# senikm/trpx

Measured on AMD Instinct MI355X. Metric: frames/s (Terse encode + Prolix decode round trip, 512x512 uint16 stack, bit-exact vs CPU ref), higher is better.
Workload: dtype u16

## Files before the change

trpx_amd/csrc/api.hip:

```cpp
#include <hip/hip_runtime.h>
#include <stdarg.h>
#include <stdio.h>
#include <stdlib.h>
#include <string.h>
#include <algorithm>
#include <vector>

#include "../../include/trpx_hip.h"
#include "encode_kernels.hpp"
#include "profile.hpp"

namespace trpx {
Profiler& profiler() {
    static thread_local Profiler p;
    return p;
}
}

namespace {

thread_local char g_err[512] = "";
thread_local bool t_force_two_pass = false;

int fail(int code, const char* fmt, ...) {
// ... 225 lines not shown
        trpx::fused_ws_forget(workspace, workspace_bytes, ws + w.fused);
        HIP_TRY(trpx::launch_encode_fused(dtype, a, ws + w.fused, static_cast<hipStream_t>(stream)));
    } else {
        trpx::fused_ws_forget(workspace, workspace_bytes);
        HIP_TRY(trpx::launch_encode(dtype, a, static_cast<hipStream_t>(stream)));
        if (index && out)
            return build_index_impl(dtype, out, out_capacity, frame_offsets, n_values, n_frames, block, index, status, false, stream);
    }
    return TRPX_OK;
}

int trpx_encode_checked(int dtype, const void* pixels, size_t n_values, size_t n_frames, unsigned block, uint8_t* out,
                        size_t out_capacity, uint64_t* frame_offsets, uint32_t* status, void* index, void* workspace,
                        size_t workspace_bytes, void* stream, uint32_t* host_status) {
    uint32_t st[TRPX_STATUS_WORDS] = {0};
    for (int attempt = 0; attempt < 2; ++attempt) {
        t_force_two_pass = attempt == 1;
        const int rc = trpx_encode_indexed(dtype, pixels, n_values, n_frames, block, out, out_capacity, frame_offsets, status,
                                           index, workspace, workspace_bytes, stream);
        t_force_two_pass = false;
        if (rc) return rc;
        HIP_TRY(hipMemcpyAsync(st, status, sizeof st, hipMemcpyDeviceToHost, static_cast<hipStream_t>(stream)));
        HIP_TRY(hipStreamSynchronize(static_cast<hipStream_t>(stream)));
        if (st[0] != TRPX_ERR_TIMEOUT) break;
    }
    if (host_status) memcpy(host_status, st, sizeof st);
    if (st[0]) return fail((int)st[0], "trpx_encode_checked: device status %u", st[0]);
    return TRPX_OK;
}

int trpx_decode(int stream_signed, int out_dtype, const uint8_t* terse, size_t terse_bytes,
                const uint64_t* frame_offsets, size_t n_values, size_t n_frames, unsigned block, void* pixels_out,
                uint32_t* status, void* workspace, size_t workspace_bytes, void* stream) {
    trpx::FrameGeom g;
    if (!trpx_dtype_size(out_dtype)) return fail(TRPX_ERR_INVALID_ARG, "trpx_decode: unknown dtype %d", out_dtype);
    if (is64(out_dtype))
        return trpx_decode_convert(stream_signed, out_dtype, terse, terse_bytes, frame_offsets, n_values, n_frames, block, pixels_out,
                                   status, workspace, workspace_bytes, stream);
    if (block == 0 || block > kMaxBlock)
        return fail(TRPX_ERR_UNSUPPORTED, "trpx_decode: block=%u (supported: 1..%u)", block, kMaxBlock);
    if ((stream_signed != 0) != (trpx_dtype_is_signed(out_dtype) != 0))
        return fail(TRPX_ERR_UNSUPPORTED, "trpx_decode: stream signed=%d into dtype %d: only same-signedness decode "
                    "is defined by the reference (Terse.hpp:356-357)", stream_signed, out_dtype);
    if (!geom_of(n_values, block, &g) || !sizes_ok(g, n_frames) || terse_bytes == 0)
        return fail(TRPX_ERR_INVALID_ARG, "trpx_decode: bad sizes");
    if (!terse || !pixels_out || !status || !workspace) return fail(TRPX_ERR_INVALID_ARG, "trpx_decode: null pointer");
    if ((uintptr_t)terse % 4 || (uintptr_t)workspace % 8 || (uintptr_t)frame_offsets % 8 || (uintptr_t)status % 8 ||
        (uintptr_t)pixels_out % trpx_dtype_size(out_dtype))
        return fail(TRPX_ERR_INVALID_ARG, "trpx_decode: misaligned pointer (terse needs 4 B, workspace 8 B)");
    const DecWs w = dec_ws(g, n_frames, trpx_dtype_size(out_dtype));
    if (workspace_bytes < w.total)
        return fail(TRPX_ERR_CAPACITY, "trpx_decode: workspace %zu < %zu", workspace_bytes, w.total);

    trpx::fused_ws_forget(workspace, workspace_bytes);
    trpx::DecodeArgs a{};
    a.terse = terse;
    a.terse_bytes = terse_bytes;
    a.frame_offsets = frame_offsets;
    a.geom = g;
    a.n_frames = (uint32_t)n_frames;
    a.pixels_out = pixels_out;
    a.status = status;
    char* ws = static_cast<char*>(workspace);
    a.walk_offsets = reinterpret_cast<uint64_t*>(ws + w.walk_offsets);
    a.tile_off = reinterpret_cast<uint64_t*>(ws + w.tile_off);
    a.widths = reinterpret_cast<uint8_t*>(ws + w.widths);
    a.seg_ws = ws + w.seg;
#ifdef TRPX_DIAGNOSTICS
    static const bool no_defer = getenv("TRPX_NO_DEFER") != nullptr;
#else
    constexpr bool no_defer = false;
#endif
    a.defer = no_defer ? nullptr : reinterpret_cast<uint32_t*>(ws + w.defer + trpx::kDeferFront);
    const int route = g_decode_path;
    const bool basic = route == 1, force_tiles = route == 2;
    const bool bits32 = 8 * (uint64_t)trpx_worst_case_bytes(out_dtype, n_values, block) < 0xF0000000ull;
    const bool fast_ok = frame_offsets && !basic && bits32 && block == (unsigned)trpx::kBlock;
    const bool frame26 = 8 * (uint64_t)trpx_worst_case_bytes(out_dtype, n_values, block) + (1u << 17) < (1ull << 26);
    a.chain = route != 4 && route != 2 && bits32;
    a.parts_per_frame = a.chain ? trpx::chain_parts_per_frame(g, n_frames, trpx_dtype_size(out_dtype)) : trpx::parts_per_frame(g, n_frames);
    const bool parts_ok = a.parts_per_frame > 1u && n_frames * (uint64_t)a.parts_per_frame < 0x7FFFFFFFull && a.defer;
    if (parts_ok) {
        a.parts = reinterpret_cast<trpx::PartDesc*>(ws + w.parts);
        a.part_ws = ws + w.part_ws;
    } else a.parts_per_frame = 1;
    if (fast_ok && (parts_ok || (frame26 && trpx::parts_per_frame(g, n_frames) == 1u)) && !force_tiles)
        HIP_TRY(trpx::launch_decode_frames(out_dtype, a, static_cast<hipStream_t>(stream)));
    else if (fast_ok)
        HIP_TRY(trpx::launch_decode_fast(out_dtype, a, false, static_cast<hipStream_t>(stream)));
    else
        HIP_TRY(trpx::launch_decode(out_dtype, a, frame_offsets != nullptr, static_cast<hipStream_t>(stream)));
    return TRPX_OK;
}

static int build_index_impl(int dtype, const uint8_t* terse, size_t terse_bytes, const uint64_t* frame_offsets,
                            size_t n_values, size_t n_frames, unsigned block, void* index, uint32_t* status,
                            bool clear_status, void* stream) {
    trpx::FrameGeom g;
    if (block != (unsigned)trpx::kBlock) return fail(TRPX_ERR_UNSUPPORTED, "trpx_build_index: the decode index needs block=12");
    if (is64(dtype)) return fail(TRPX_ERR_UNSUPPORTED, "trpx_build_index: no decode index for 64-bit containers (generic kernels)");
    if (!trpx_dtype_size(dtype) || !geom_of(n_values, block, &g) || !sizes_ok(g, n_frames) || !terse_bytes)
        return fail(TRPX_ERR_INVALID_ARG, "trpx_build_index: bad dtype/sizes");
    if (!terse || !frame_offsets || !index || !status) return fail(TRPX_ERR_INVALID_ARG, "trpx_build_index: null pointer");
    if ((uintptr_t)terse % 4 || (uintptr_t)index % 16 || (uintptr_t)frame_offsets % 8 || (uintptr_t)status % 8)
        return fail(TRPX_ERR_INVALID_ARG, "trpx_build_index: misaligned pointer");
    if (8 * (uint64_t)trpx_worst_case_bytes(dtype, n_values, block) >= 0xF0000000ull)
        return fail(TRPX_ERR_UNSUPPORTED, "trpx_build_index: frames of >= 2^32 bits");
    const IdxLayout il = idx_layout(g, n_frames, trpx_dtype_size(dtype));
    trpx::DecodeArgs a{};
    a.terse = terse;
    a.terse_bytes = terse_bytes;
    a.frame_offsets = frame_offsets;
    a.geom = g;
    a.n_frames = (uint32_t)n_frames;
    a.status = status;
    a.tile_off = reinterpret_cast<uint64_t*>(static_cast<char*>(index) + il.group_off);
    a.widths = reinterpret_cast<uint8_t*>(static_cast<char*>(index) + il.widths);
    a.seg_ws = static_cast<char*>(index) + il.seg;
    a.defer = reinterpret_cast<uint32_t*>(static_cast<char*>(index) + il.defer + trpx::kDeferFront);
    a.index_per_frame = 8 * (uint64_t)trpx_worst_case_bytes(dtype, n_values, block) + (1u << 17) < (1ull << 26) && g_decode_path != 2;
    a.parts_per_frame = trpx::chain_parts_per_frame(g, n_frames, trpx_dtype_size(dtype));
    a.chain = a.parts_per_frame > 1u && n_frames * (uint64_t)a.parts_per_frame < 0x7FFFFFFFull && g_decode_path != 2 && g_decode_path != 4;
    if (a.chain) {
        a.parts = reinterpret_cast<trpx::PartDesc*>(static_cast<char*>(index) + il.parts);
        a.part_ws = static_cast<char*>(index) + il.part_ws;
    } else a.parts_per_frame = 1;
    HIP_TRY(trpx::launch_walk_only(a, (uint32_t)(8 * trpx_dtype_size(dtype)), clear_status, static_cast<hipStream_t>(stream)));
    return TRPX_OK;
}

int trpx_build_index(int dtype, const uint8_t* terse, size_t terse_bytes, const uint64_t* frame_offsets,
                     size_t n_values, size_t n_frames, unsigned block, void* index, uint32_t* status, void* stream) {
    return build_index_impl(dtype, terse, terse_bytes, frame_offsets, n_values, n_frames, block, index, status, true, stream);
}

int trpx_decode_indexed(int stream_signed, int out_dtype, const uint8_t* terse, size_t terse_bytes,
                        const uint64_t* frame_offsets, const void* index, size_t n_values, size_t n_frames,
                        unsigned block, void* pixels_out, uint32_t* status, void* stream) {
    trpx::FrameGeom g;
    if (!trpx_dtype_size(out_dtype)) return fail(TRPX_ERR_INVALID_ARG, "trpx_decode_indexed: unknown dtype %d", out_dtype);
    if (block != (unsigned)trpx::kBlock) return fail(TRPX_ERR_UNSUPPORTED, "trpx_decode_indexed: block=%u", block);
// ... 579 lines not shown
```

trpx_amd/csrc/codec_common.hpp:

```cpp
#pragma once
#include <hip/hip_runtime.h>
#include <stdint.h>

namespace trpx {

constexpr int kBlock = 12;
constexpr int kWave = 64;
constexpr int kThreads = 256;
constexpr int kTileBlocks = kThreads;
constexpr int kTileValues = kTileBlocks * kBlock;

struct FrameGeom {
    uint64_t n_values;
    uint32_t n_blocks;
    uint32_t n_tiles;
    uint32_t block;
};

template <typename T> struct PixelTraits;
template <> struct PixelTraits<uint8_t>  { using U = uint8_t;  static constexpr int bits = 8;  static constexpr bool is_signed = false; };
template <> struct PixelTraits<int8_t>   { using U = uint8_t;  static constexpr int bits = 8;  static constexpr bool is_signed = true;  };
template <> struct PixelTraits<uint16_t> { using U = uint16_t; static constexpr int bits = 16; static constexpr bool is_signed = false; };
template <> struct PixelTraits<int16_t>  { using U = uint16_t; static constexpr int bits = 16; static constexpr bool is_signed = true;  };
template <> struct PixelTraits<uint32_t> { using U = uint32_t; static constexpr int bits = 32; static constexpr bool is_signed = false; };
// ... 49 lines not shown
        return s < 0 ? 0u - (uint32_t)s : (uint32_t)s;
    }
    return (uint32_t)(typename PixelTraits<T>::U)v;
}

__device__ __forceinline__ uint32_t wave_inclusive_scan(uint32_t v) {
    v += (uint32_t)__builtin_amdgcn_update_dpp(0, (int)v, 0x111, 0xf, 0xf, false);
    v += (uint32_t)__builtin_amdgcn_update_dpp(0, (int)v, 0x112, 0xf, 0xf, false);
    v += (uint32_t)__builtin_amdgcn_update_dpp(0, (int)v, 0x114, 0xf, 0xf, false);
    v += (uint32_t)__builtin_amdgcn_update_dpp(0, (int)v, 0x118, 0xf, 0xf, false);
    v += (uint32_t)__builtin_amdgcn_update_dpp(0, (int)v, 0x142, 0xa, 0xf, false);
    v += (uint32_t)__builtin_amdgcn_update_dpp(0, (int)v, 0x143, 0xc, 0xf, false);
    return v;
}

__device__ __forceinline__ uint32_t wave_max(uint32_t v) {
    auto step = [](uint32_t x, uint32_t y) { return x > y ? x : y; };
    v = step(v, (uint32_t)__builtin_amdgcn_update_dpp(0, (int)v, 0x111, 0xf, 0xf, false));
    v = step(v, (uint32_t)__builtin_amdgcn_update_dpp(0, (int)v, 0x112, 0xf, 0xf, false));
    v = step(v, (uint32_t)__builtin_amdgcn_update_dpp(0, (int)v, 0x114, 0xf, 0xf, false));
    v = step(v, (uint32_t)__builtin_amdgcn_update_dpp(0, (int)v, 0x118, 0xf, 0xf, false));
    v = step(v, (uint32_t)__builtin_amdgcn_update_dpp(0, (int)v, 0x142, 0xa, 0xf, false));
    v = step(v, (uint32_t)__builtin_amdgcn_update_dpp(0, (int)v, 0x143, 0xc, 0xf, false));
    return (uint32_t)__builtin_amdgcn_readlane((int)v, 63);
}

__device__ __forceinline__ int lane_id() { return (int)(threadIdx.x & 63u); }
__device__ __forceinline__ int wave_id() { return __builtin_amdgcn_readfirstlane((int)(threadIdx.x >> 6)); }

__device__ __forceinline__ uint32_t block_exclusive_scan(uint32_t v, uint32_t* wave_tot, uint32_t* total) {
    uint32_t inc = wave_inclusive_scan(v);
    if (lane_id() == 63) wave_tot[wave_id()] = inc;
    __syncthreads();
    uint32_t t0 = wave_tot[0], t1 = wave_tot[1], t2 = wave_tot[2], t3 = wave_tot[3];
    int w = wave_id();
    uint32_t base = (w > 0 ? t0 : 0u) + (w > 1 ? t1 : 0u) + (w > 2 ? t2 : 0u);
    *total = t0 + t1 + t2 + t3;
    return base + inc - v;
}

template <int kUnused = 0>
__global__ __launch_bounds__(kThreads) void k_zero_words(uint64_t* __restrict__ p, uint64_t n, uint64_t* __restrict__ q,
                                                         uint64_t m) {
    for (uint64_t i = (uint64_t)blockIdx.x * kThreads + threadIdx.x; i < n; i += (uint64_t)gridDim.x * kThreads) p[i] = 0ull;
    if (blockIdx.x == 0 && threadIdx.x < m) q[threadIdx.x] = 0ull;
}
inline void zero_status(uint32_t* status, hipStream_t st) {
    hipLaunchKernelGGL(k_zero_words<0>, dim3(1), dim3(kThreads), 0, st, static_cast<uint64_t*>(nullptr), (uint64_t)0,
                       reinterpret_cast<uint64_t*>(status), (uint64_t)4);
}

__host__ __device__ inline uint64_t align_up(uint64_t x, uint64_t a) { return (x + a - 1) / a * a; }
constexpr uint32_t kDeferSlots = 64, kDeferSlotWords = 16;
constexpr size_t kDeferFront = 8u * kDeferSlots * kDeferSlotWords;
inline size_t defer_bytes(size_t n_frames) { return kDeferFront + align_up(4 * (n_frames + 2), 256); }

}
```

trpx_amd/csrc/decode_frame.hip:

```cpp
#include "codec_common.hpp"
#include "encode_kernels.hpp"
#include "profile.hpp"
#include "unpack_common.hpp"

namespace trpx {

#ifndef TRPX_FRAME_WAVES
#define TRPX_FRAME_WAVES 4
#endif
constexpr int kFrameWaves = TRPX_FRAME_WAVES;
constexpr int kFrameThreads = kFrameWaves * kWave;

#ifndef TRPX_FRAME_CHUNK_DW
#define TRPX_FRAME_CHUNK_DW 2048
#endif
#ifndef TRPX_IDX_TOUCH
#define TRPX_IDX_TOUCH 1
#endif
template <typename T>
struct FrameCfg {
#ifdef TRPX_FRAME_GPW
    static constexpr int kGpw = TRPX_FRAME_GPW;
#else
    static constexpr int kGpw = 4;
#endif
    static constexpr int kStepGroups = (kFrameWaves - 1) * kGpw;
    static constexpr int kStepBlocks = kStepGroups * kWave;
    static constexpr int kChunkDw = TRPX_FRAME_CHUNK_DW;
#ifdef TRPX_DEC_DIRECT_STORES
    static constexpr bool kOutStaged = sizeof(T) == 4;
#else
    static constexpr bool kOutStaged = true;
#endif
    static constexpr int kRawDw = 4 * RawQuads<T>::n;
    static constexpr int kOutDw = kWave * kBlock * (int)sizeof(T) / 4;
    static_assert(kChunkDw % (kWave * 4) == 0, "window = whole 1 KB pieces");
};

__device__ __forceinline__ void lds_dma16(const uint32_t* src_uniform, uint32_t lane_byte_offset, uint32_t lds_base) {
    uint32_t keep;
    asm volatile("s_mov_b32 %0, m0\n\ts_mov_b32 m0, %3\n\ts_nop 0\n\tglobal_load_lds_dwordx4 %1, %2\n\ts_mov_b32 m0, %0"
                 : "=&s"(keep) : "v"(lane_byte_offset), "s"(src_uniform), "s"(lds_base) : "memory");
}

template <typename T, int MODE, bool PARTS = false, bool LINES = false>
__device__ __forceinline__ void decode_frame_body(const uint8_t* __restrict__ terse, uint64_t terse_bytes,
                                                  const uint64_t* __restrict__ frame_offsets, const FrameGeom& g,
                                                  T* __restrict__ pixels_out, uint32_t* __restrict__ defer,
                                                  uint32_t* __restrict__ status, const uint64_t item,
                                                  const uint8_t* __restrict__ idx_widths, const uint64_t* __restrict__ idx_group_off,
                                                  const PartDesc* __restrict__ parts = nullptr) {
    using Cfg = FrameCfg<T>;
    constexpr bool IDX = MODE == 1;
    constexpr int kStepBlocks = Cfg::kStepBlocks, kChunkDw = Cfg::kChunkDw;
    constexpr uint32_t kMaxW = PixelTraits<T>::bits;
    __shared__ __attribute__((aligned(16))) uint32_t s_chunk[kChunkDw + 4];
    constexpr int kPosEntries = kStepBlocks + 64 + 68;
    __shared__ uint32_t s_pos[2][kPosEntries];
    uint32_t* const s_posx = &s_pos[0][0];
    constexpr uint32_t kPosBits = 26, kPosMask = (1u << kPosBits) - 1u;
    __shared__ __attribute__((aligned(16))) uint32_t s_out[kFrameWaves - 1][Cfg::kOutStaged ? Cfg::kOutDw + kStageCarryDw : 4];
    __shared__ uint32_t s_err;
#ifdef TRPX_DEC_LDS_PAD
    __shared__ uint32_t s_pad[TRPX_DEC_LDS_PAD / 4];
    if (terse_bytes == 1) s_pad[threadIdx.x] = 0;
#endif
    __shared__ uint32_t s_role[kFrameWaves];
    __shared__ uint64_t s_keep[3];

    const uint32_t lane = (uint32_t)lane_id();
    const int hw_wave = wave_id();
    uint64_t frame = item;
    uint32_t pb0 = 0, pb1 = g.n_blocks, ppos0 = 0, pw0 = 0, ppos1 = 0, pw1 = 0;
    if constexpr (PARTS && MODE == 1) {
        const uint32_t unit_blocks = (uint32_t)(uintptr_t)parts;
        const uint32_t upf = (g.n_blocks + unit_blocks - 1u) / unit_blocks;
        frame = item / upf;
        pb0 = (uint32_t)(item % upf) * unit_blocks;
        pb1 = pb0 + unit_blocks < g.n_blocks ? pb0 + unit_blocks : g.n_blocks;
        ppos0 = (uint32_t)idx_group_off[frame * g.n_tiles + pb0 / (uint32_t)kTileBlocks];
        pw0 = pb0 ? (uint32_t)idx_widths[frame * g.n_blocks + pb0 - 1u] : 0u;
        if (pb1 < g.n_blocks) {
            ppos1 = (uint32_t)idx_group_off[frame * g.n_tiles + pb1 / (uint32_t)kTileBlocks];
            pw1 = (uint32_t)idx_widths[frame * g.n_blocks + pb1 - 1u];
        }
    } else if constexpr (PARTS) {
        const PartDesc d = parts[item];
        frame = d.frame; pb0 = d.b0; pb1 = d.b1; ppos0 = d.pos0; pw0 = d.w0; ppos1 = d.pos1; pw1 = d.w1;
        if (pb1 <= pb0) return;
    }
    const uint64_t fo = frame_offsets[frame], fe = frame_offsets[frame + 1];
    if (threadIdx.x == 0) {
        s_err = (fe > fo && fe <= terse_bytes && (uint64_t)ppos0 < 8 * (fe - fo) && pb1 <= g.n_blocks) ? 0u : 1u;
        s_keep[0] = (uint64_t)(uintptr_t)status; s_keep[1] = (uint64_t)(uintptr_t)defer; s_keep[2] = item;
    }
    uint32_t hw_slot = 0;
    {
        uint32_t hwid;
        asm volatile("s_getreg_b32 %0, hwreg(HW_REG_HW_ID)" : "=s"(hwid));
        if (lane == 0) s_role[hw_wave] = ((hwid >> 4) & 3u) == (hwid & 3u) ? 1u : 0u;
        hw_slot = hwid & 7u;
    }
    __syncthreads();
    int walker_wave = 0;
#pragma unroll
    for (int i = kFrameWaves - 1; i >= 0; --i) walker_wave = s_role[i] ? i : walker_wave;
    walker_wave = __builtin_amdgcn_readfirstlane(walker_wave);
    const int wave = (hw_wave - walker_wave + kFrameWaves) % kFrameWaves;
    if (s_err) {
        if (threadIdx.x == 0) atomicMax(&status[0], 5u);
        return;
    }
    const uint32_t* __restrict__ s32 = reinterpret_cast<const uint32_t*>(terse);
    const uint64_t n_dw = (terse_bytes + 3) / 4;
    const bool base16 = ((uintptr_t)terse & 15) == 0;
    const uint64_t frame_abit = 8 * fo + ppos0;
    const uint32_t limit = (uint32_t)(8 * (fe - fo) - ppos0);
    const uint64_t frame_dw = frame_abit >> 5;
    const uint32_t frame_sh = (uint32_t)(frame_abit & 31);
    const uint32_t n_blocks = pb1 - pb0;
    const bool at_end = pb1 == g.n_blocks;
    const uint32_t nb_last = at_end ? (uint32_t)(g.n_values - (uint64_t)(g.n_blocks - 1) * kBlock) : (uint32_t)kBlock;
    const uint32_t sb0 = defer ? (uint32_t)((kFrameWaves - 1) * kWave) : (uint32_t)kStepBlocks;
    const uint32_t n_steps = n_blocks <= sb0 ? 1u : 1u + (n_blocks - sb0 + kStepBlocks - 1) / kStepBlocks;
    auto step_begin = [&](uint32_t t) -> uint32_t { return t == 0u ? 0u : sb0 + (t - 1u) * kStepBlocks; };
    T* __restrict__ fout = pixels_out + frame * g.n_values + (uint64_t)pb0 * kBlock;
    const uint32_t out_c = LINES ? (uint32_t)((uintptr_t)fout & 127u) : 0u;

#ifdef TRPX_DEC_NO_STORE
    uint32_t diag_acc = 0;
#endif
    int32_t c_lo = 0, c_hi = 0;
    uint32_t b = 0, w_prev = pw0, pos = 0;
#ifndef TRPX_DEC_WALK_PRIO
#define TRPX_DEC_WALK_PRIO 3
#endif
#ifndef TRPX_DEFER_NUM
#define TRPX_DEFER_NUM 2
#define TRPX_DEFER_DEN 9
#endif
    if (wave == 0) __builtin_amdgcn_s_setprio(TRPX_DEC_WALK_PRIO);
    constexpr int kIdxChunks = IDX ? kStepBlocks / kWave : 1;
    constexpr int kIdxQuads = IDX ? kStepBlocks / (4 * kWave) : 1;
    static_assert(!IDX || kStepBlocks % (4 * kWave) == 0, "the width prefetch covers a super-step in whole quads of 64 lanes (TRPX_FRAME_GPW: a multiple of 4 per three extraction waves)");
    __shared__ __attribute__((aligned(4))) uint8_t s_wnext[IDX ? kStepBlocks : 4];
    [[maybe_unused]] auto idx_load = [&](uint32_t ss, uint32_t (&dst)[kIdxQuads]) {
        const uint8_t* __restrict__ wfl = idx_widths + frame * g.n_blocks + pb0;
        const uint32_t bb = step_begin(ss), be = step_begin(ss + 1u) < n_blocks ? step_begin(ss + 1u) : n_blocks;
#pragma unroll
        for (int j = 0; j < kIdxQuads; ++j) {
            const uint32_t bi = bb + 4u * ((uint32_t)j * kWave + lane);
            uint32_t v = 0u;
            if (bi + 4u <= be) __builtin_memcpy(&v, wfl + bi, 4);
            else {
#pragma unroll
                for (uint32_t k = 0; k < 4u; ++k) v |= bi + k < be ? (uint32_t)wfl[bi + k] << (8u * k) : 0u;
            }
            dst[j] = v;
        }
    };
    [[maybe_unused]] auto idx_park = [&](const uint32_t (&src)[kIdxQuads]) {
#pragma unroll
        for (int j = 0; j < kIdxQuads; ++j) reinterpret_cast<uint32_t*>(s_wnext)[j * kWave + lane] = src[j];
    };
    if constexpr (IDX) {
// ... 373 lines not shown
                        uint32_t ss = sq;
                        asm volatile("" : "+v"(ss));
                        if (mine) UnpackRegsDispatch<T, 0, PixelTraits<T>::bits>::run(raw, ss, wd, o);
                        todo &= ~__ballot(mine);
                    }
#ifdef TRPX_DEC_NO_STORE
                    if (full) diag_acc ^= o[0];
#else
                    if (full) store_packed<T>(dst, o);
#endif
                }
                if (blk + 1 == n_blocks && blk < step1 && !full) {
                    const uint32_t mask = w >= 32u ? 0xFFFFFFFFu : ((1u << w) - 1u);
                    uint32_t p = q;
                    for (uint32_t k = 0; k < nb_last; ++k) {
                        uint32_t f = 0;
                        if (w) {
                            const uint64_t d = frame_dw + (p >> 5);
                            const uint64_t two = (uint64_t)(d < n_dw ? s32[d] : 0u) | ((uint64_t)(d + 1 < n_dw ? s32[d + 1] : 0u) << 32);
                            f = (uint32_t)(two >> (p & 31u)) & mask;
                            if (PixelTraits<T>::is_signed) f = (uint32_t)((int32_t)(f << (32u - w)) >> (32u - w));
                        }
                        dst[k] = (T)f;
                        p += w;
                    }
                }
            }
        }
#ifdef TRPX_DEC_STAMPS
        { const uint64_t t1 = __builtin_readcyclecounter(); st_work += t1 - st_t0; st_t0 = t1; }
#endif
        __syncthreads();
#ifdef TRPX_DEC_STAMPS
        { const uint64_t t1 = __builtin_readcyclecounter(); st_wait += t1 - st_t0; st_t0 = t1; }
#endif
        if (s_err) break;
    }
#ifdef TRPX_DEC_STAMPS
    if (lane == 0) {
        uint32_t hwid;
        asm volatile("s_getreg_b32 %0, hwreg(HW_REG_HW_ID)" : "=s"(hwid));
        uint32_t* dbg = reinterpret_cast<uint32_t*>(fout) + 8 * wave;
        dbg[0] = (uint32_t)st_work; dbg[1] = (uint32_t)st_wait; dbg[2] = hwid; dbg[3] = (uint32_t)(st_t0 - st_start);
        dbg[4] = (uint32_t)(st_start & 0xFFFFFFFFu);
        uint32_t xcc;
        asm volatile("s_getreg_b32 %0, hwreg(HW_REG_XCC_ID)" : "=s"(xcc));
        dbg[5] = xcc;
        dbg[6] = dbg[7] = 0;
    }
#endif
#ifdef TRPX_DEC_NO_STORE
    if (diag_acc == 0x12345678u) fout[threadIdx.x] = (T)diag_acc;
#endif
    if (threadIdx.x == 0 && s_err != 0u) {
        asm volatile("" ::: "memory");
        uint32_t* const status_l = reinterpret_cast<uint32_t*>((uintptr_t)s_keep[0]);
        uint32_t* const defer_l = reinterpret_cast<uint32_t*>((uintptr_t)s_keep[1]);
        if (s_err == 1u) atomicMax(&status_l[0], 5u);
        if (s_err >= 2u) {
            defer_l[1u + atomicAdd(&defer_l[0], 1u)] = (uint32_t)s_keep[2] | (s_err == 3u ? 0x80000000u : 0u);
            if (s_err == 3u) atomicAdd(reinterpret_cast<unsigned long long*>(defer_l) - 2, 1ull);
        }
    }
}

template <typename T, bool LINES>
__global__ __launch_bounds__(kFrameThreads, sizeof(T) == 4 ? 6 : 8) void k_decode_frames(const uint8_t* __restrict__ terse, uint64_t terse_bytes,
                                                               const uint64_t* __restrict__ frame_offsets, FrameGeom g,
                                                               T* __restrict__ pixels_out, uint32_t* __restrict__ defer,
                                                               uint32_t* __restrict__ status) {
    decode_frame_body<T, 0, false, LINES>(terse, terse_bytes, frame_offsets, g, pixels_out, defer, status, blockIdx.x, nullptr, nullptr);
}

template <typename T>
__global__ __launch_bounds__(kFrameThreads, sizeof(T) == 4 ? 6 : 8) void k_decode_parts(const uint8_t* __restrict__ terse, uint64_t terse_bytes,
                                                               const uint64_t* __restrict__ frame_offsets, FrameGeom g,
                                                               T* __restrict__ pixels_out, uint32_t* __restrict__ status,
                                                               const PartDesc* __restrict__ parts, const uint32_t* __restrict__ frame_mode) {
    if (status[0] != 0u) return;
    if (frame_mode && frame_mode[parts[blockIdx.x].frame] != 0u) return;
    decode_frame_body<T, 0, true, true>(terse, terse_bytes, frame_offsets, g, pixels_out, nullptr, status, blockIdx.x, nullptr, nullptr, parts);
}

template <typename T>
__global__ __launch_bounds__(kFrameThreads, sizeof(T) == 4 ? 6 : 8) void k_decode_frames_indexed(const uint8_t* __restrict__ terse, uint64_t terse_bytes,
                                                               const uint64_t* __restrict__ frame_offsets, FrameGeom g,
                                                               const uint8_t* __restrict__ widths, const uint64_t* __restrict__ group_off,
                                                               const uint32_t* __restrict__ list, T* __restrict__ pixels_out,
                                                               uint32_t* __restrict__ status) {
    uint64_t frame = blockIdx.x;
    if (list) {
        if (blockIdx.x >= list[0] || status[0] != 0u) return;
        frame = list[1u + blockIdx.x] & 0x7FFFFFFFu;
    }
#ifdef TRPX_IDX_LINES
    decode_frame_body<T, 1, false, true>(terse, terse_bytes, frame_offsets, g, pixels_out, nullptr, status, frame, widths, group_off);
#else
    decode_frame_body<T, 1>(terse, terse_bytes, frame_offsets, g, pixels_out, nullptr, status, frame, widths, group_off);
#endif
}

template <typename T>
__global__ __launch_bounds__(kFrameThreads, sizeof(T) == 4 ? 6 : 8) void k_decode_units_indexed(const uint8_t* __restrict__ terse, uint64_t terse_bytes,
                                                               const uint64_t* __restrict__ frame_offsets, FrameGeom g,
                                                               const uint8_t* __restrict__ widths, const uint64_t* __restrict__ group_off,
                                                               uint32_t unit_blocks, T* __restrict__ pixels_out, uint32_t* __restrict__ status,
                                                               const uint32_t* __restrict__ frame_mode) {
    if (status[0] != 0u) return;
    if (frame_mode && frame_mode[blockIdx.x / ((g.n_blocks + unit_blocks - 1u) / unit_blocks)] == 0u) return;
    decode_frame_body<T, 1, true>(terse, terse_bytes, frame_offsets, g, pixels_out, nullptr, status, blockIdx.x, widths, group_off,
                                  reinterpret_cast<const PartDesc*>((uintptr_t)unit_blocks));
}
template <typename T>
static uint32_t units_choose(const DecodeArgs& a, uint64_t* cost_out);
template <typename T>
static hipError_t launch_decode_units_indexed_t(const DecodeArgs& a, hipStream_t st, const uint32_t* frame_mode) {
    const uint32_t unit_blocks = units_choose<T>(a, nullptr);
    const uint32_t upf = (a.geom.n_blocks + unit_blocks - 1u) / unit_blocks;
    hipLaunchKernelGGL((k_decode_units_indexed<T>), dim3(a.n_frames * upf), dim3(kFrameThreads), 0, st, a.terse, (uint64_t)a.terse_bytes,
                       a.frame_offsets, a.geom, static_cast<const uint8_t*>(a.widths), static_cast<const uint64_t*>(a.tile_off), unit_blocks,
                       static_cast<T*>(a.pixels_out), a.status, frame_mode);
    return hipGetLastError();
}
constexpr uint64_t units_resident(size_t pixel_bytes) { return (uint64_t)(pixel_bytes == 4 ? 6 : 8) * 256u; }
// ... 31 lines not shown
                                                               uint32_t* __restrict__ defer, uint32_t* __restrict__ status) {
    decode_frame_body<T, 2>(terse, terse_bytes, frame_offsets, g, static_cast<T*>(nullptr), defer, status, blockIdx.x, widths, group_off);
}

hipError_t launch_index_frames(uint32_t max_w, const DecodeArgs& a, bool clear_status, hipStream_t st) {
    hipLaunchKernelGGL(k_zero_words<0>, dim3(1), dim3(kThreads), 0, st, reinterpret_cast<uint64_t*>(a.defer) - kDeferSlots * kDeferSlotWords,
                       (uint64_t)(kDeferSlots * kDeferSlotWords + 1), reinterpret_cast<uint64_t*>(a.status), (uint64_t)(clear_status ? 4 : 0));
    if (max_w <= 8u)
        hipLaunchKernelGGL((k_index_frames<uint8_t>), dim3(a.n_frames), dim3(kFrameThreads), 0, st, a.terse, (uint64_t)a.terse_bytes,
                           a.frame_offsets, a.geom, a.widths, a.tile_off, a.defer, a.status);
    else if (max_w <= 16u)
        hipLaunchKernelGGL((k_index_frames<uint16_t>), dim3(a.n_frames), dim3(kFrameThreads), 0, st, a.terse, (uint64_t)a.terse_bytes,
                           a.frame_offsets, a.geom, a.widths, a.tile_off, a.defer, a.status);
    else
        hipLaunchKernelGGL((k_index_frames<uint32_t>), dim3(a.n_frames), dim3(kFrameThreads), 0, st, a.terse, (uint64_t)a.terse_bytes,
                           a.frame_offsets, a.geom, a.widths, a.tile_off, a.defer, a.status);
    return launch_seg_listed(a, max_w, st);
}

template <typename T>
static hipError_t launch_decode_frames_indexed_t(const DecodeArgs& a, const uint32_t* list, hipStream_t st) {
#ifdef TRPX_IDX_AS_UNITS
    if (!list) return launch_decode_units_indexed_t<T>(a, st, nullptr);
#endif
    if (!list && a.geom.n_blocks > 8u * FrameCfg<T>::kStepBlocks) {
        uint64_t cost_units = 0;
        units_choose<T>(a, &cost_units);
        const uint64_t resident = units_resident(sizeof(T));
        const uint64_t cost_whole = ((a.n_frames + resident - 1) / resident) * ((uint64_t)a.geom.n_blocks + FrameCfg<T>::kStepBlocks);
        if (10u * cost_units < 9u * cost_whole) return launch_decode_units_indexed_t<T>(a, st, nullptr);
    }
    hipLaunchKernelGGL((k_decode_frames_indexed<T>), dim3(a.n_frames), dim3(kFrameThreads), 0, st, a.terse, (uint64_t)a.terse_bytes,
                       a.frame_offsets, a.geom, static_cast<const uint8_t*>(a.widths), static_cast<const uint64_t*>(a.tile_off), list,
                       static_cast<T*>(a.pixels_out), a.status);
    return hipGetLastError();
}

hipError_t launch_decode_frames_indexed(int dtype, const DecodeArgs& a, const uint32_t* list, hipStream_t st) {
    switch (dtype) {
    case 0: return launch_decode_frames_indexed_t<uint8_t>(a, list, st);
    case 1: return launch_decode_frames_indexed_t<int8_t>(a, list, st);
    case 2: return launch_decode_frames_indexed_t<uint16_t>(a, list, st);
    case 3: return launch_decode_frames_indexed_t<int16_t>(a, list, st);
    case 4: return launch_decode_frames_indexed_t<uint32_t>(a, list, st);
    case 5: return launch_decode_frames_indexed_t<int32_t>(a, list, st);
    }
    return hipErrorInvalidValue;
}

template <typename T>
static hipError_t launch_decode_frames_t(const DecodeArgs& a, hipStream_t st) {
    uint32_t* defer = a.defer && a.seg_ws ? a.defer : nullptr;
    const bool chain = a.chain && a.parts && a.parts_per_frame > 1u;
    if (chain) {
        if (!defer) return hipErrorInvalidValue;
        const hipError_t e = launch_chain_zero(a, (uint32_t)PixelTraits<T>::bits, true, st);
        if (e != hipSuccess) return e;
    } else
        hipLaunchKernelGGL(k_zero_words<0>, dim3(1), dim3(kThreads), 0, st,
                           defer ? reinterpret_cast<uint64_t*>(defer) - kDeferSlots * kDeferSlotWords : static_cast<uint64_t*>(nullptr),
                           (uint64_t)(defer ? kDeferSlots * kDeferSlotWords + 1 : 0),
                           reinterpret_cast<uint64_t*>(a.status), (uint64_t)4);
    Profiler& prof = profiler();
    prof.begin();
    prof.mark(st);
    if (chain) {
        if (!defer) return hipErrorInvalidValue;
        constexpr int dt = PixelTraits<T>::bits == 8 ? (PixelTraits<T>::is_signed ? 1 : 0)
                           : PixelTraits<T>::bits == 16 ? (PixelTraits<T>::is_signed ? 3 : 2) : (PixelTraits<T>::is_signed ? 5 : 4);
        constexpr bool narrow = sizeof(T) < 4;
        const uint32_t* frame_mode = nullptr;
        hipError_t e = launch_build_index_chain(a, (uint32_t)PixelTraits<T>::bits, narrow, &frame_mode, st);
        if (e != hipSuccess) return e;
        prof.mark(st);
        e = launch_seg_listed(a, (uint32_t)PixelTraits<T>::bits, st);
        if (e != hipSuccess) return e;
#ifdef TRPX_CHAIN_EXTRACT_TILES
        const bool tiles = TRPX_CHAIN_EXTRACT_TILES != 0;
#else
        const bool tiles = sizeof(T) == 4 || a.geom.n_blocks < (1u << 18);
#endif
        e = tiles ? launch_unpack_tiles(dt, a, st, narrow ? frame_mode : nullptr) : launch_decode_units_indexed(dt, a, st, narrow ? frame_mode : nullptr);
        if (e != hipSuccess) return e;
        if constexpr (narrow)
            hipLaunchKernelGGL((k_decode_parts<T>), dim3(a.n_frames * a.parts_per_frame), dim3(kFrameThreads), 0, st, a.terse, (uint64_t)a.terse_bytes,
                               a.frame_offsets, a.geom, static_cast<T*>(a.pixels_out), a.status, static_cast<const PartDesc*>(a.parts), frame_mode);
        prof.mark(st);
        return hipGetLastError();
    } else if (a.parts && a.parts_per_frame > 1u) {
        if (!defer) return hipErrorInvalidValue;
        const hipError_t e = launch_build_parts(a, (uint32_t)PixelTraits<T>::bits, st);
        if (e != hipSuccess) return e;
        hipLaunchKernelGGL((k_decode_parts<T>), dim3(a.n_frames * a.parts_per_frame), dim3(kFrameThreads), 0, st, a.terse, (uint64_t)a.terse_bytes,
                           a.frame_offsets, a.geom, static_cast<T*>(a.pixels_out), a.status, static_cast<const PartDesc*>(a.parts),
                           static_cast<const uint32_t*>(nullptr));
    } else if ((a.geom.n_values * sizeof(T)) % 128u == 0u && (uintptr_t)a.pixels_out % 128u == 0u)
        hipLaunchKernelGGL((k_decode_frames<T, false>), dim3(a.n_frames), dim3(kFrameThreads), 0, st, a.terse, (uint64_t)a.terse_bytes,
                           a.frame_offsets, a.geom, static_cast<T*>(a.pixels_out), defer, a.status);
    else
        hipLaunchKernelGGL((k_decode_frames<T, true>), dim3(a.n_frames), dim3(kFrameThreads), 0, st, a.terse, (uint64_t)a.terse_bytes,
                           a.frame_offsets, a.geom, static_cast<T*>(a.pixels_out), defer, a.status);
    prof.mark(st);
    if (defer) {
        const hipError_t e = launch_decode_deferred(PixelTraits<T>::bits == 8 ? (PixelTraits<T>::is_signed ? 1 : 0)
                                                    : PixelTraits<T>::bits == 16 ? (PixelTraits<T>::is_signed ? 3 : 2)
                                                                                 : (PixelTraits<T>::is_signed ? 5 : 4), a, st);
        prof.mark(st);
        if (e != hipSuccess) return e;
    }
    return hipGetLastError();
}

hipError_t launch_decode_frames(int dtype, const DecodeArgs& a, hipStream_t st) {
    switch (dtype) {
    case 0: return launch_decode_frames_t<uint8_t>(a, st);
    case 1: return launch_decode_frames_t<int8_t>(a, st);
    case 2: return launch_decode_frames_t<uint16_t>(a, st);
    case 3: return launch_decode_frames_t<int16_t>(a, st);
    case 4: return launch_decode_frames_t<uint32_t>(a, st);
    case 5: return launch_decode_frames_t<int32_t>(a, st);
    }
    return hipErrorInvalidValue;
}

}
```

trpx_amd/csrc/encode_fused.hip:

```cpp
#include <stddef.h>
#include <utility>
#include "codec_common.hpp"
#include "encode_kernels.hpp"
#include "profile.hpp"
#include <stdlib.h>
#include <mutex>
#include <vector>

namespace trpx {

#ifndef TRPX_FUSED_SUB32
#define TRPX_FUSED_SUB32 5
#endif
#ifndef TRPX_FUSED_SUB16
#define TRPX_FUSED_SUB16 4
#endif
template <typename T> constexpr int sub_tiles() { return sizeof(T) <= 2 ? TRPX_FUSED_SUB16 : TRPX_FUSED_SUB32; }
#ifndef TRPX_FUSED_OCC16
#define TRPX_FUSED_OCC16 8
#endif
#ifndef TRPX_FUSED_OCC32
#define TRPX_FUSED_OCC32 4
#endif
template <typename T> constexpr int fused_occupancy() { return sizeof(T) == 1 ? 8 : (sizeof(T) == 2 ? TRPX_FUSED_OCC16 : TRPX_FUSED_OCC32); }
// ... 763 lines not shown
    __syncthreads();
    if (threadIdx.x == 0) {
        uint32_t m = s_max[0];
        for (int i = 1; i < 4; ++i) m = s_max[i] > m ? s_max[i] : m;
        if (m) atomicMax(&status[1], m);
    }
    for (uint64_t i = b; i < n_frame_words; i += (uint64_t)gridDim.x * kThreads) frame_words[i] = 0ull;
    if (b == 0 && ws_tag) ws_tag[0] = tag;
    if (b >= n_tiles) return;
    tile_desc[b] = 0ull;
    if (failed || b == 0) { xw[b] = 0ull; return; }
    if (!(pw & kBndHead)) { xw[b] = 0ull; return; }
    const uint64_t d = pw & kPosMask;
    if (b > 1 && (pb & kBndHead) && (pb & kPosMask) == d) return;
    uint32_t acc = (uint32_t)xb;
    xw[b] = 0ull;
    for (uint64_t k = b + 1; k < n_tiles; ++k) {
        const uint64_t pk = pos[k];
        if (!((pk & kBndHead) && (pk & kPosMask) == d)) break;
        acc |= (uint32_t)xw[k];
        xw[k] = 0ull;
    }
    if (4 * d + 4 <= out_capacity) out32[d] = acc;
}

template <typename T>
static uint32_t fused_tiles_per_frame(const FrameGeom& g) {
    constexpr uint32_t tb = sub_tiles<T>() * kThreads;
    return (g.n_blocks + tb - 1) / tb;
}

size_t fused_workspace_bytes(const FrameGeom& g, size_t n_frames) {
    const size_t tpf = ((size_t)g.n_blocks + 2 * kThreads - 1) / (2 * kThreads);
    return align_up(8 * (3 * n_frames * tpf + 16 * ((size_t)kAccLines + 1) * n_frames + 1), 256) + 64 * n_frames * tpf;
}

namespace {
struct CleanSig {
    uint32_t elem, tiles_per_frame, n_frames, n_blocks;
    bool operator==(const CleanSig& o) const { return elem == o.elem && tiles_per_frame == o.tiles_per_frame && n_frames == o.n_frames && n_blocks == o.n_blocks; }
};
struct CleanWs { int device; const void* ptr; CleanSig sig; uint64_t tag; };
std::mutex g_clean_mu;
std::vector<CleanWs> g_clean;
uint64_t g_next_tag = 0x5452505800000001ull;
}
void fused_ws_forget(const void* lo, size_t bytes, const void* keep) {
    std::lock_guard<std::mutex> lk(g_clean_mu);
    const char* a = static_cast<const char*>(lo);
    for (size_t i = 0; i < g_clean.size();) {
        const char* p = static_cast<const char*>(g_clean[i].ptr);
        if (p != keep && (!lo || (p >= a && p < a + bytes))) { g_clean[i] = g_clean.back(); g_clean.pop_back(); } else ++i;
    }
}

template <typename T>
static hipError_t launch_fused_t(const EncodeArgs& e, void* ws, hipStream_t st) {
    FusedArgs a;
    a.g = e.geom;
    a.n_frames = e.n_frames;
    a.tiles_per_frame = fused_tiles_per_frame<T>(e.geom);
    a.out_capacity = e.out_capacity;
    const size_t tiles = (size_t)e.n_frames * a.tiles_per_frame;
    a.tile_desc = static_cast<uint64_t*>(ws);
    a.tail_desc = a.tile_desc + tiles;
    a.bnd_pos = a.tail_desc + tiles;
    a.n_acc = fused_acc_lines(a.tiles_per_frame);
    a.acc_stride = 16u * a.n_acc;
    a.frame_acc = a.bnd_pos + tiles;
    a.frame_pref = a.frame_acc + 1;
    a.frame_base = a.frame_acc + (size_t)a.acc_stride * e.n_frames;
    a.frame_offsets = e.frame_offsets;
    a.out32 = reinterpret_cast<uint32_t*>(e.out);
    a.status = e.status;
    a.idx_widths = e.idx_widths;
    a.idx_group_off = e.idx_group_off;
    const size_t frame_words = 16 * ((size_t)a.n_acc + 1) * e.n_frames;
    uint64_t* const frame_words_base = a.frame_acc;
    a.ws_tag = frame_words_base + frame_words;
    a.stamps = reinterpret_cast<uint64_t*>(static_cast<char*>(ws) + align_up(8 * (3 * tiles + frame_words + 1), 256));
#ifdef TRPX_DIAGNOSTICS
    a.debug = getenv("TRPX_FUSED_DEBUG") ? (uint32_t)atoi(getenv("TRPX_FUSED_DEBUG")) : 0u;
#else
    a.debug = 0u;
#endif
    hipStreamCaptureStatus cap = hipStreamCaptureStatusNone;
    if (hipStreamIsCapturing(st, &cap) != hipSuccess) { (void)hipGetLastError(); cap = hipStreamCaptureStatusActive; }
    const bool capturing = cap != hipStreamCaptureStatusNone;
    int device = -1;
    (void)hipGetDevice(&device);
    const CleanSig sig{(uint32_t)sizeof(T), a.tiles_per_frame, e.n_frames, e.geom.n_blocks};
    uint64_t expect = 0, tag = 0;
    if (!capturing) {
        std::lock_guard<std::mutex> lk(g_clean_mu);
        tag = g_next_tag++;
        for (size_t i = 0; i < g_clean.size(); ++i)
            if (g_clean[i].device == device && g_clean[i].ptr == ws) {
                if (g_clean[i].sig == sig) expect = g_clean[i].tag;
                g_clean[i] = g_clean.back(); g_clean.pop_back();
                break;
            }
    }
    a.expect_tag = expect;
    Profiler& prof = profiler();
    prof.begin();
    prof.mark(st);
// ... 39 lines not shown
```

trpx_amd/csrc/encode_kernels.hpp:

```cpp
#pragma once
#include <hip/hip_runtime.h>
#include <stdint.h>
#include <stddef.h>
#include "codec_common.hpp"

namespace trpx {

struct EncodeArgs {
    const void* pixels;
    FrameGeom   geom;
    uint32_t    n_frames;
    uint8_t*    out;
    size_t      out_capacity;
    uint64_t*   frame_offsets;
    uint32_t*   status;
    uint64_t*   frame_size;
    uint64_t*   tile_off;
    uint32_t*   tile_bits;
    uint8_t*    idx_widths;
    uint64_t*   idx_group_off;
};

struct PartDesc {
    uint32_t frame, b0, b1, pos0, w0, pos1, w1, pad;
};
constexpr uint32_t kPartBlocks = 16384;
constexpr uint32_t kPartMaxBlocks = 32768;
constexpr uint32_t kManyFrames = 768;
constexpr uint32_t kManyBlocks = 1u << 20;
uint32_t single_part_blocks(size_t n_frames);
void set_single_part_rule(uint32_t many_frames, uint32_t many_blocks);

struct DecodeArgs {
    const uint8_t*  terse;
    size_t          terse_bytes;
    const uint64_t* frame_offsets;
    FrameGeom       geom;
    uint32_t        n_frames;
    void*           pixels_out;
    uint32_t*       status;
    uint64_t*       tile_off;
    uint8_t*        widths;
    uint64_t*       walk_offsets;
    uint32_t*       defer;
    void*           seg_ws;
    bool            index_per_frame = false;
    PartDesc*       parts = nullptr;
    uint32_t        parts_per_frame = 1;
    void*           part_ws = nullptr;
    bool            index_given = false;
    bool            chain = false;
};
uint32_t parts_per_frame(const FrameGeom& g, size_t n_frames);
size_t part_workspace_bytes(const FrameGeom& g, size_t n_frames);
hipError_t launch_build_parts(const DecodeArgs& a, uint32_t max_w, hipStream_t st);
uint32_t chain_parts_per_frame(const FrameGeom& g, size_t n_frames, size_t pixel_bytes);
size_t chain_workspace_bytes(const FrameGeom& g, size_t n_frames, size_t pixel_bytes);
hipError_t launch_build_index_chain(const DecodeArgs& a, uint32_t max_w, bool narrow, const uint32_t** frame_mode, hipStream_t st);
hipError_t launch_chain_zero(const DecodeArgs& a, uint32_t max_w, bool clear_status, hipStream_t st);
hipError_t launch_unpack_tiles(int dtype, const DecodeArgs& a, hipStream_t st, const uint32_t* frame_mode = nullptr);

hipError_t launch_encode(int dtype, const EncodeArgs& a, hipStream_t st);
hipError_t launch_encode_generic(int dtype, const EncodeArgs& a, hipStream_t st);
size_t fused_workspace_bytes(const FrameGeom& g, size_t n_frames);
hipError_t launch_encode_fused(int dtype, const EncodeArgs& a, void* ws, hipStream_t st);
void fused_ws_forget(const void* lo, size_t bytes, const void* keep = nullptr);
hipError_t launch_decode(int dtype, const DecodeArgs& a, bool have_offsets, hipStream_t st);
hipError_t launch_decode_convert(int dtype, const DecodeArgs& a, int stream_signed, bool have_offsets, hipStream_t st);
hipError_t launch_decode_fast(int dtype, const DecodeArgs& a, bool have_index, hipStream_t st, bool per_frame = false);
hipError_t launch_decode_frames(int dtype, const DecodeArgs& a, hipStream_t st);
hipError_t launch_decode_frames_indexed(int dtype, const DecodeArgs& a, const uint32_t* list, hipStream_t st);
hipError_t launch_decode_units_indexed(int dtype, const DecodeArgs& a, hipStream_t st, const uint32_t* frame_mode = nullptr);
hipError_t launch_index_frames(uint32_t max_w, const DecodeArgs& a, bool clear_status, hipStream_t st);
hipError_t launch_seg_listed(const DecodeArgs& a, uint32_t max_w, hipStream_t st);
hipError_t launch_seg_groups(const DecodeArgs& a, uint32_t max_w, const uint64_t* states, hipStream_t st);
hipError_t launch_walk_only(const DecodeArgs& a, uint32_t max_w, bool clear_status, hipStream_t st);
hipError_t launch_walk_serial(const DecodeArgs& a, uint32_t max_w, hipStream_t st);
hipError_t launch_index_group_states(const DecodeArgs& a, uint64_t* states, hipStream_t st);
hipError_t launch_walk_groups(const DecodeArgs& a, uint32_t max_w, const uint64_t* states, bool clear_status, hipStream_t st);
size_t seg_workspace_bytes(const FrameGeom& g, size_t n_frames);
size_t dense_workspace_bytes(const FrameGeom& g, size_t n_frames);
hipError_t launch_dense_listed(const DecodeArgs& a, uint32_t max_w, void* dense_ws, const uint32_t* list, hipStream_t st);
void set_dense_route(bool on);
hipError_t launch_seg_walk(const DecodeArgs& a, uint32_t max_w, hipStream_t st);
bool seg_single_wave(const FrameGeom& g, size_t n_frames);
hipError_t launch_decode_deferred(int dtype, const DecodeArgs& a, hipStream_t st);
hipError_t launch_synth(int dtype, uint64_t seed, uint64_t frame0, size_t n_frames, size_t n_values,
                        void* out, hipStream_t st);

}
```

Baseline: 3.803 million.

## Fold decode defer-workspace zeroing into the frame kernel's last-arriving block

Removes the separate k_zero_words launch before the frame decode kernel when the workspace is known clean, tracked by a host-side tag registry. The last block to arrive, counted with a packed 64-bit atomic counter, resets the defer slots and status and writes a tag. A later call can skip zeroing if the tag matches, and falls back to a device-side reset when it does not. This saves one kernel launch per decode call. The cost is added atomic traffic, host mutex bookkeeping, and stale-tag correctness risks.

```diff
diff --git a/trpx_amd/csrc/api.hip b/trpx_amd/csrc/api.hip
--- a/trpx_amd/csrc/api.hip
+++ b/trpx_amd/csrc/api.hip
@@ -301,6 +301,13 @@
     if (workspace_bytes < w.total)
         return fail(TRPX_ERR_CAPACITY, "trpx_decode: workspace %zu < %zu", workspace_bytes, w.total);
 
+    char* ws = static_cast<char*>(workspace);
+    hipStreamCaptureStatus cap = hipStreamCaptureStatusNone;
+    if (hipStreamIsCapturing(static_cast<hipStream_t>(stream), &cap) != hipSuccess) { (void)hipGetLastError(); cap = hipStreamCaptureStatusActive; }
+    const bool capturing = cap != hipStreamCaptureStatusNone;
+    const uint32_t ws_elem = 0x100u + (uint32_t)trpx_dtype_size(out_dtype);
+    uint64_t ws_expect = 0, ws_tag = 0;
+    if (!capturing) ws_expect = trpx::clean_ws_take(ws + w.defer, ws_elem, (uint32_t)n_frames, g.n_blocks, &ws_tag);
     trpx::fused_ws_forget(workspace, workspace_bytes);
     trpx::DecodeArgs a{};
     a.terse = terse;
@@ -310,7 +317,11 @@
     a.n_frames = (uint32_t)n_frames;
     a.pixels_out = pixels_out;
     a.status = status;
-    char* ws = static_cast<char*>(workspace);
+    bool ws_clean = false;
+    a.ws_expect = ws_expect;
+    a.ws_tag = ws_tag;
+    a.ws_capturing = capturing;
+    a.ws_clean_out = &ws_clean;
     a.walk_offsets = reinterpret_cast<uint64_t*>(ws + w.walk_offsets);
     a.tile_off = reinterpret_cast<uint64_t*>(ws + w.tile_off);
     a.widths = reinterpret_cast<uint8_t*>(ws + w.widths);
@@ -333,9 +344,10 @@
         a.parts = reinterpret_cast<trpx::PartDesc*>(ws + w.parts);
         a.part_ws = ws + w.part_ws;
     } else a.parts_per_frame = 1;
-    if (fast_ok && (parts_ok || (frame26 && trpx::parts_per_frame(g, n_frames) == 1u)) && !force_tiles)
+    if (fast_ok && (parts_ok || (frame26 && trpx::parts_per_frame(g, n_frames) == 1u)) && !force_tiles) {
         HIP_TRY(trpx::launch_decode_frames(out_dtype, a, static_cast<hipStream_t>(stream)));
-    else if (fast_ok)
+        if (ws_clean && !capturing) trpx::clean_ws_put(ws + w.defer, ws_elem, (uint32_t)n_frames, g.n_blocks, ws_tag);
+    } else if (fast_ok)
         HIP_TRY(trpx::launch_decode_fast(out_dtype, a, false, static_cast<hipStream_t>(stream)));
     else
         HIP_TRY(trpx::launch_decode(out_dtype, a, frame_offsets != nullptr, static_cast<hipStream_t>(stream)));
diff --git a/trpx_amd/csrc/codec_common.hpp b/trpx_amd/csrc/codec_common.hpp
--- a/trpx_amd/csrc/codec_common.hpp
+++ b/trpx_amd/csrc/codec_common.hpp
@@ -125,6 +125,7 @@
 
 __host__ __device__ inline uint64_t align_up(uint64_t x, uint64_t a) { return (x + a - 1) / a * a; }
 constexpr uint32_t kDeferSlots = 64, kDeferSlotWords = 16;
+constexpr int kDeferTagOff = 5, kDeferArriveOff = 22;
 constexpr size_t kDeferFront = 8u * kDeferSlots * kDeferSlotWords;
 inline size_t defer_bytes(size_t n_frames) { return kDeferFront + align_up(4 * (n_frames + 2), 256); }
 
diff --git a/trpx_amd/csrc/decode_frame.hip b/trpx_amd/csrc/decode_frame.hip
--- a/trpx_amd/csrc/decode_frame.hip
+++ b/trpx_amd/csrc/decode_frame.hip
@@ -43,13 +43,52 @@
                  : "=&s"(keep) : "v"(lane_byte_offset), "s"(src_uniform), "s"(lds_base) : "memory");
 }
 
+constexpr uint64_t kWsLegacy = ~0ull;
+constexpr uint32_t kArriveBits = 21;
+__device__ __forceinline__ uint64_t* defer_word(uint32_t* defer, int off) { return reinterpret_cast<uint64_t*>(defer) - off; }
+__device__ __forceinline__ void frames_exit(uint32_t ws_mode, uint32_t err, uint32_t* status, uint32_t* defer, uint32_t item, uint64_t tag) {
+    if (ws_mode == 0u) {
+        if (err == 1u) atomicMax(&status[0], 5u);
+        if (err >= 2u) {
+            defer[1u + atomicAdd(&defer[0], 1u)] = item | (err == 3u ? 0x80000000u : 0u);
+            if (err == 3u) atomicAdd(reinterpret_cast<unsigned long long*>(defer) - 2, 1ull);
+        }
+        return;
+    }
+    uint64_t* const slots = reinterpret_cast<uint64_t*>(defer) - kDeferSlots * kDeferSlotWords;
+    if (ws_mode == 2u) {
+        __hip_atomic_store(&status[0], 7u, __ATOMIC_RELAXED, __HIP_MEMORY_SCOPE_AGENT);
+        if (item == 0u) {
+            for (uint32_t i = 0; i <= kDeferSlots * kDeferSlotWords; ++i)
+                if (i != kDeferSlots * kDeferSlotWords - kDeferTagOff) __hip_atomic_store(slots + i, 0ull, __ATOMIC_RELAXED, __HIP_MEMORY_SCOPE_AGENT);
+            if (tag) __hip_atomic_store(defer_word(defer, kDeferTagOff), tag, __ATOMIC_RELAXED, __HIP_MEMORY_SCOPE_AGENT);
+        }
+        return;
+    }
+    constexpr uint64_t one = 1ull, mask = (one << kArriveBits) - 1ull;
+    const uint64_t add = one | (err >= 2u ? one << kArriveBits : 0ull) | (err == 1u ? one << (2 * kArriveBits) : 0ull);
+    const uint64_t before = __hip_atomic_fetch_add(defer_word(defer, kDeferArriveOff), add, __ATOMIC_RELAXED, __HIP_MEMORY_SCOPE_AGENT);
+    if (err >= 2u) defer[1u + (uint32_t)((before >> kArriveBits) & mask)] = item | (err == 3u ? 0x80000000u : 0u);
+    if ((uint32_t)(before & mask) + 1u != gridDim.x) return;
+    const uint64_t sum = before + add;
+    defer[0] = (uint32_t)((sum >> kArriveBits) & mask);
+    reinterpret_cast<uint2*>(status)[0] = make_uint2((sum >> (2 * kArriveBits)) != 0ull ? 5u : 0u, 0u);
+    reinterpret_cast<uint2*>(status)[1] = make_uint2(0u, 0u);
+    reinterpret_cast<uint2*>(status)[2] = make_uint2(0u, 0u);
+    reinterpret_cast<uint2*>(status)[3] = make_uint2(0u, 0u);
+    for (uint32_t i = 0; i < kDeferSlots; ++i) __hip_atomic_store(slots + i * kDeferSlotWords, 0ull, __ATOMIC_RELAXED, __HIP_MEMORY_SCOPE_AGENT);
+    __hip_atomic_store(defer_word(defer, kDeferArriveOff), 0ull, __ATOMIC_RELAXED, __HIP_MEMORY_SCOPE_AGENT);
+    if (tag) __hip_atomic_store(defer_word(defer, kDeferTagOff), tag, __ATOMIC_RELAXED, __HIP_MEMORY_SCOPE_AGENT);
+}
+
 template <typename T, int MODE, bool PARTS = false, bool LINES = false>
 __device__ __forceinline__ void decode_frame_body(const uint8_t* __restrict__ terse, uint64_t terse_bytes,
                                                   const uint64_t* __restrict__ frame_offsets, const FrameGeom& g,
                                                   T* __restrict__ pixels_out, uint32_t* __restrict__ defer,
                                                   uint32_t* __restrict__ status, const uint64_t item,
                                                   const uint8_t* __restrict__ idx_widths, const uint64_t* __restrict__ idx_group_off,
-                                                  const PartDesc* __restrict__ parts = nullptr) {
+                                                  const PartDesc* __restrict__ parts = nullptr, uint64_t ws_expect = kWsLegacy,
+                                                  uint64_t ws_tag = 0) {
     using Cfg = FrameCfg<T>;
     constexpr bool IDX = MODE == 1;
     constexpr int kStepBlocks = Cfg::kStepBlocks, kChunkDw = Cfg::kChunkDw;
@@ -66,7 +105,8 @@
     if (terse_bytes == 1) s_pad[threadIdx.x] = 0;
 #endif
     __shared__ uint32_t s_role[kFrameWaves];
-    __shared__ uint64_t s_keep[3];
+    __shared__ uint64_t s_keep[4];
+    __shared__ uint32_t s_wsmode;
 
     const uint32_t lane = (uint32_t)lane_id();
     const int hw_wave = wave_id();
@@ -92,7 +132,11 @@
     const uint64_t fo = frame_offsets[frame], fe = frame_offsets[frame + 1];
     if (threadIdx.x == 0) {
         s_err = (fe > fo && fe <= terse_bytes && (uint64_t)ppos0 < 8 * (fe - fo) && pb1 <= g.n_blocks) ? 0u : 1u;
-        s_keep[0] = (uint64_t)(uintptr_t)status; s_keep[1] = (uint64_t)(uintptr_t)defer; s_keep[2] = item;
+        s_keep[0] = (uint64_t)(uintptr_t)status; s_keep[1] = (uint64_t)(uintptr_t)defer; s_keep[2] = item; s_keep[3] = ws_tag;
+        uint32_t m = 0u;
+        if (MODE == 0 && !PARTS && defer && ws_expect != kWsLegacy)
+            m = ws_expect == 0ull || __hip_atomic_load(defer_word(defer, kDeferTagOff), __ATOMIC_RELAXED, __HIP_MEMORY_SCOPE_AGENT) == ws_expect ? 1u : 2u;
+        s_wsmode = m;
     }
     uint32_t hw_slot = 0;
     {
@@ -108,9 +152,10 @@
     walker_wave = __builtin_amdgcn_readfirstlane(walker_wave);
     const int wave = (hw_wave - walker_wave + kFrameWaves) % kFrameWaves;
     if (s_err) {
-        if (threadIdx.x == 0) atomicMax(&status[0], 5u);
+        if (threadIdx.x == 0) frames_exit(s_wsmode, 1u, status, defer, (uint32_t)item, ws_tag);
         return;
     }
+    if (s_wsmode == 2u) defer = nullptr;
     const uint32_t* __restrict__ s32 = reinterpret_cast<const uint32_t*>(terse);
     const uint64_t n_dw = (terse_bytes + 3) / 4;
     const bool base16 = ((uintptr_t)terse & 15) == 0;
@@ -590,15 +635,10 @@
 #ifdef TRPX_DEC_NO_STORE
     if (diag_acc == 0x12345678u) fout[threadIdx.x] = (T)diag_acc;
 #endif
-    if (threadIdx.x == 0 && s_err != 0u) {
+    if (threadIdx.x == 0 && (s_err != 0u || s_wsmode != 0u)) {
         asm volatile("" ::: "memory");
-        uint32_t* const status_l = reinterpret_cast<uint32_t*>((uintptr_t)s_keep[0]);
-        uint32_t* const defer_l = reinterpret_cast<uint32_t*>((uintptr_t)s_keep[1]);
-        if (s_err == 1u) atomicMax(&status_l[0], 5u);
-        if (s_err >= 2u) {
-            defer_l[1u + atomicAdd(&defer_l[0], 1u)] = (uint32_t)s_keep[2] | (s_err == 3u ? 0x80000000u : 0u);
-            if (s_err == 3u) atomicAdd(reinterpret_cast<unsigned long long*>(defer_l) - 2, 1ull);
-        }
+        frames_exit(s_wsmode, s_err, reinterpret_cast<uint32_t*>((uintptr_t)s_keep[0]), reinterpret_cast<uint32_t*>((uintptr_t)s_keep[1]),
+                    (uint32_t)s_keep[2], s_keep[3]);
     }
 }
 
@@ -606,8 +646,9 @@
 __global__ __launch_bounds__(kFrameThreads, sizeof(T) == 4 ? 6 : 8) void k_decode_frames(const uint8_t* __restrict__ terse, uint64_t terse_bytes,
                                                                const uint64_t* __restrict__ frame_offsets, FrameGeom g,
                                                                T* __restrict__ pixels_out, uint32_t* __restrict__ defer,
-                                                               uint32_t* __restrict__ status) {
-    decode_frame_body<T, 0, false, LINES>(terse, terse_bytes, frame_offsets, g, pixels_out, defer, status, blockIdx.x, nullptr, nullptr);
+                                                               uint32_t* __restrict__ status, uint64_t ws_expect, uint64_t ws_tag) {
+    decode_frame_body<T, 0, false, LINES>(terse, terse_bytes, frame_offsets, g, pixels_out, defer, status, blockIdx.x, nullptr, nullptr,
+                                          nullptr, ws_expect, ws_tag);
 }
 
 template <typename T>
@@ -745,10 +786,22 @@
 static hipError_t launch_decode_frames_t(const DecodeArgs& a, hipStream_t st) {
     uint32_t* defer = a.defer && a.seg_ws ? a.defer : nullptr;
     const bool chain = a.chain && a.parts && a.parts_per_frame > 1u;
+    bool fold = defer && !chain && !(a.parts && a.parts_per_frame > 1u) && a.n_frames < (1u << kArriveBits) && seg_single_wave(a.geom, a.n_frames);
+#ifdef TRPX_DEFER_STATS
+    fold = false;
+#endif
+    const uint64_t expect = fold ? a.ws_expect : kWsLegacy;
     if (chain) {
         if (!defer) return hipErrorInvalidValue;
         const hipError_t e = launch_chain_zero(a, (uint32_t)PixelTraits<T>::bits, true, st);
         if (e != hipSuccess) return e;
+    } else if (fold) {
+        if (expect == 0) {
+            uint64_t* const slots = reinterpret_cast<uint64_t*>(defer) - kDeferSlots * kDeferSlotWords;
+            constexpr uint64_t n = kDeferSlots * kDeferSlotWords + 1, t = kDeferSlots * kDeferSlotWords - kDeferTagOff;
+            if (a.ws_capturing) hipLaunchKernelGGL(k_zero_words<0>, dim3(1), dim3(kThreads), 0, st, slots, t, slots + t + 1, n - t - 1);
+            else hipLaunchKernelGGL(k_zero_words<0>, dim3(1), dim3(kThreads), 0, st, slots, n, static_cast<uint64_t*>(nullptr), (uint64_t)0);
+        }
     } else
         hipLaunchKernelGGL(k_zero_words<0>, dim3(1), dim3(kThreads), 0, st,
                            defer ? reinterpret_cast<uint64_t*>(defer) - kDeferSlots * kDeferSlotWords : static_cast<uint64_t*>(nullptr),
@@ -789,11 +842,12 @@
                            static_cast<const uint32_t*>(nullptr));
     } else if ((a.geom.n_values * sizeof(T)) % 128u == 0u && (uintptr_t)a.pixels_out % 128u == 0u)
         hipLaunchKernelGGL((k_decode_frames<T, false>), dim3(a.n_frames), dim3(kFrameThreads), 0, st, a.terse, (uint64_t)a.terse_bytes,
-                           a.frame_offsets, a.geom, static_cast<T*>(a.pixels_out), defer, a.status);
+                           a.frame_offsets, a.geom, static_cast<T*>(a.pixels_out), defer, a.status, expect, fold ? a.ws_tag : 0ull);
     else
         hipLaunchKernelGGL((k_decode_frames<T, true>), dim3(a.n_frames), dim3(kFrameThreads), 0, st, a.terse, (uint64_t)a.terse_bytes,
-                           a.frame_offsets, a.geom, static_cast<T*>(a.pixels_out), defer, a.status);
+                           a.frame_offsets, a.geom, static_cast<T*>(a.pixels_out), defer, a.status, expect, fold ? a.ws_tag : 0ull);
     prof.mark(st);
+    if (fold && a.ws_tag && a.ws_clean_out && hipPeekAtLastError() == hipSuccess) *a.ws_clean_out = true;
     if (defer) {
         const hipError_t e = launch_decode_deferred(PixelTraits<T>::bits == 8 ? (PixelTraits<T>::is_signed ? 1 : 0)
                                                     : PixelTraits<T>::bits == 16 ? (PixelTraits<T>::is_signed ? 3 : 2)
diff --git a/trpx_amd/csrc/encode_fused.hip b/trpx_amd/csrc/encode_fused.hip
--- a/trpx_amd/csrc/encode_fused.hip
+++ b/trpx_amd/csrc/encode_fused.hip
@@ -839,6 +839,28 @@
         const char* p = static_cast<const char*>(g_clean[i].ptr);
         if (p != keep && (!lo || (p >= a && p < a + bytes))) { g_clean[i] = g_clean.back(); g_clean.pop_back(); } else ++i;
     }
+}
+
+uint64_t clean_ws_take(const void* ptr, uint32_t elem, uint32_t n_frames, uint32_t n_blocks, uint64_t* new_tag) {
+    int device = -1;
+    (void)hipGetDevice(&device);
+    const CleanSig sig{elem, 0u, n_frames, n_blocks};
+    std::lock_guard<std::mutex> lk(g_clean_mu);
+    *new_tag = g_next_tag++;
+    for (size_t i = 0; i < g_clean.size(); ++i)
+        if (g_clean[i].device == device && g_clean[i].ptr == ptr) {
+            const uint64_t t = g_clean[i].sig == sig ? g_clean[i].tag : 0ull;
+            g_clean[i] = g_clean.back(); g_clean.pop_back();
+            return t;
+        }
+    return 0ull;
+}
+void clean_ws_put(const void* ptr, uint32_t elem, uint32_t n_frames, uint32_t n_blocks, uint64_t tag) {
+    int device = -1;
+    (void)hipGetDevice(&device);
+    std::lock_guard<std::mutex> lk(g_clean_mu);
+    if (g_clean.size() >= 64) g_clean.erase(g_clean.begin());
+    g_clean.push_back(CleanWs{device, ptr, CleanSig{elem, 0u, n_frames, n_blocks}, tag});
 }
 
 template <typename T>
diff --git a/trpx_amd/csrc/encode_kernels.hpp b/trpx_amd/csrc/encode_kernels.hpp
--- a/trpx_amd/csrc/encode_kernels.hpp
+++ b/trpx_amd/csrc/encode_kernels.hpp
@@ -50,6 +50,9 @@
     void*           part_ws = nullptr;
     bool            index_given = false;
     bool            chain = false;
+    uint64_t        ws_expect = 0, ws_tag = 0;
+    bool            ws_capturing = false;
+    bool*           ws_clean_out = nullptr;
 };
 uint32_t parts_per_frame(const FrameGeom& g, size_t n_frames);
 size_t part_workspace_bytes(const FrameGeom& g, size_t n_frames);
@@ -65,6 +68,8 @@
 size_t fused_workspace_bytes(const FrameGeom& g, size_t n_frames);
 hipError_t launch_encode_fused(int dtype, const EncodeArgs& a, void* ws, hipStream_t st);
 void fused_ws_forget(const void* lo, size_t bytes, const void* keep = nullptr);
+uint64_t clean_ws_take(const void* ptr, uint32_t elem, uint32_t n_frames, uint32_t n_blocks, uint64_t* new_tag);
+void clean_ws_put(const void* ptr, uint32_t elem, uint32_t n_frames, uint32_t n_blocks, uint64_t tag);
 hipError_t launch_decode(int dtype, const DecodeArgs& a, bool have_offsets, hipStream_t st);
 hipError_t launch_decode_convert(int dtype, const DecodeArgs& a, int stream_signed, bool have_offsets, hipStream_t st);
 hipError_t launch_decode_fast(int dtype, const DecodeArgs& a, bool have_index, hipStream_t st, bool per_frame = false);
```

Result: no change. 3.777 million (median of 6 runs) (-0.7%).
